# ZhengkunTian/OpenTransformer

Measured on AMD Instinct MI355X. Metric: utterances/sec (80-d fbank, ~1000 frames) train fwd+bwd, higher is better.
Workload: dtype fp16; 1 GPU; AISHELL-1 transformer_baseline.yaml (+input_size 80), 12 enc / 6 dec layers, B=32/GPU x 1000 frames x 80-d fbank, 15 decoder rows, V=4234, residual_dropout 0.1; step = fwd + bwd + grad all-reduce + clip/Adam/Noam; global_batch=32, frames=1000, parallelism=dp1, hipgraph=True

## Files before the change

### opentransformer_amd/csrc/common.h

```cpp
#pragma once
#include <hip/hip_runtime.h>
#include <stdint.h>

#include "../../include/otrans_hip.h"

#ifdef OTR_HALF_FP16
typedef _Float16 otr_hreal;
#define OTR_H16 OTR_F16
#else
typedef __bf16 otr_hreal;
#define OTR_H16 OTR_BF16
#endif
typedef __attribute__((ext_vector_type(8))) otr_hreal bf16x8;
typedef __attribute__((ext_vector_type(2))) otr_hreal bf16x2;
typedef __attribute__((ext_vector_type(4))) float f32x4;
typedef __attribute__((ext_vector_type(2))) float f32x2;
typedef uint16_t bf16_t;

void otr_set_error(const char* fmt, ...);
int32_t otr_check_launch(const char* what);
void otr_zero_f32(float* p, int64_t n, hipStream_t s);
#define OTR_REQUIRE(cond, ...)          \
  do {                                  \
    if (!(cond)) {                      \
      otr_set_error(__VA_ARGS__);       \
      return -1;                        \
    }                                   \
  } while (0)

extern int g_otr_force_tile;
extern int g_otr_force_ksplit;
extern int g_otr_conv2_wgrad256;
extern int g_otr_attn_enc96;
extern int g_otr_wgrad256;
extern int g_otr_wgrad256_grid;
extern int g_otr_conv2_dgrad_wide;
extern int g_otr_conv2_wide;
extern int g_otr_conv2_fwd_direct;
extern int g_otr_attn_enc;
extern int g_otr_attn_xmap;
extern int g_otr_attn_bwd_split;
extern int g_otr_beam_reg;
extern int g_otr_decode_attn64;
extern int g_otr_dec_group;
extern int g_otr_ffn_map;
extern int g_otr_ffn_coh_only;
extern int g_otr_spin_limit;
extern int32_t* g_otr_fault;
extern unsigned long long* g_otr_trace;

typedef uint32_t otr_u32x4 __attribute__((ext_vector_type(4)));
typedef uint32_t otr_u32x2 __attribute__((ext_vector_type(2)));
#define OTR_GLOBAL __attribute__((address_space(1)))
__device__ __forceinline__ uint4 ld_global_b128(const void* p) {
  otr_u32x4 v = *(const OTR_GLOBAL otr_u32x4*)(p);
  return make_uint4(v.x, v.y, v.z, v.w);
}
__device__ __forceinline__ uint2 ld_global_b64(const void* p) {
  otr_u32x2 v = *(const OTR_GLOBAL otr_u32x2*)(p);
  return make_uint2(v.x, v.y);
}
__device__ __forceinline__ void st_global_b128(void* p, uint4 v) {
  otr_u32x4 t = {v.x, v.y, v.z, v.w};
  *(OTR_GLOBAL otr_u32x4*)(p) = t;
}

__device__ __forceinline__ void st_global_b128_nt(void* p, uint4 v) {
  otr_u32x4 t = {v.x, v.y, v.z, v.w};
#if defined(OTR_ST_WT) && OTR_ST_WT
  asm volatile("global_store_dwordx4 %0, %1, off sc0 sc1 nt\n\ts_nop 1" ::"v"(p), "v"(t) : "memory");
#else
  __builtin_nontemporal_store(t, (OTR_GLOBAL otr_u32x4*)(p));
#endif
}

#ifdef OTR_HALF_FP16
__device__ __forceinline__ float bf2f(bf16_t v) { return (float)__builtin_bit_cast(_Float16, v); }
__device__ __forceinline__ float h2f_lo(uint32_t w) { return bf2f((bf16_t)(w & 0xffffu)); }
__device__ __forceinline__ float h2f_hi(uint32_t w) { return bf2f((bf16_t)(w >> 16)); }
#else
__device__ __forceinline__ float bf2f(bf16_t v) { return __uint_as_float(((uint32_t)v) << 16); }
__device__ __forceinline__ float h2f_lo(uint32_t w) { return __uint_as_float(w << 16); }
__device__ __forceinline__ float h2f_hi(uint32_t w) { return __uint_as_float(w & 0xffff0000u); }
#endif
__device__ __forceinline__ bf16_t f2bf(float f) {
  otr_hreal h = (otr_hreal)f;
  return __builtin_bit_cast(bf16_t, h);
}
__device__ __forceinline__ uint32_t pack2bf(float lo, float hi) {
  f32x2 v = {lo, hi};
  bf16x2 h = __builtin_convertvector(v, bf16x2);
  return __builtin_bit_cast(uint32_t, h);
}

__device__ __forceinline__ float h2f(bf16_t v) { return bf2f(v); }
__device__ __forceinline__ bf16_t f2h(float f) { return f2bf(f); }
__device__ __forceinline__ uint32_t pack2h(float lo, float hi) { return pack2bf(lo, hi); }

typedef __attribute__((ext_vector_type(16))) float f32x16;
__device__ __forceinline__ void mma32(f32x16& acc, const uint4& a, const uint4& b) {
#ifdef OTR_HALF_FP16
  acc = __builtin_amdgcn_mfma_f32_32x32x16_f16(__builtin_bit_cast(bf16x8, a), __builtin_bit_cast(bf16x8, b), acc, 0, 0, 0);
#else
  acc = __builtin_amdgcn_mfma_f32_32x32x16_bf16(__builtin_bit_cast(bf16x8, a), __builtin_bit_cast(bf16x8, b), acc, 0, 0, 0);
#endif
}

#ifdef OTR_HALF_FP16
#define OTR_MFMA32_OP "v_mfma_f32_32x32x16_f16"
#else
#define OTR_MFMA32_OP "v_mfma_f32_32x32x16_bf16"
#endif
__device__ __forceinline__ void mma32_agpr_b(f32x16& acc, const otr_u32x4& a, const otr_u32x4& b_acc) {
  asm volatile("s_nop 1\n\t" OTR_MFMA32_OP " %0, %1, %2, %0" : "+v"(acc) : "v"(a), "a"(b_acc));
}
__device__ __forceinline__ void mma32_agpr_a(f32x16& acc, const otr_u32x4& a_acc, const otr_u32x4& b) {
  asm volatile("s_nop 1\n\t" OTR_MFMA32_OP " %0, %1, %2, %0" : "+v"(acc) : "a"(a_acc), "v"(b));
}

typedef __attribute__((address_space(3))) unsigned char lds_byte;

template <bool NT = false> __device__ __forceinline__ void lds_dma(const void* src, uint32_t lds_dst) {
  uint32_t keep;
  if constexpr (NT)
    asm volatile("s_mov_b32 %0, m0\n\ts_mov_b32 m0, %2\n\ts_nop 0\n\tglobal_load_lds_dwordx4 %1, off nt\n\ts_mov_b32 m0, %0"
                 : "=&s"(keep) : "v"(src), "s"(lds_dst) : "memory");
  else
    asm volatile("s_mov_b32 %0, m0\n\ts_mov_b32 m0, %2\n\ts_nop 0\n\tglobal_load_lds_dwordx4 %1, off\n\ts_mov_b32 m0, %0"
                 : "=&s"(keep) : "v"(src), "s"(lds_dst) : "memory");
}
__device__ __forceinline__ void lds_dma_sbase(const void* uniform_src, uint32_t lane_off, uint32_t lds_dst) {
  uint32_t keep;
  asm volatile("s_mov_b32 %0, m0\n\ts_mov_b32 m0, %3\n\ts_nop 0\n\tglobal_load_lds_dwordx4 %1, %2\n\ts_mov_b32 m0, %0"
               : "=&s"(keep) : "v"(lane_off), "s"(uniform_src), "s"(lds_dst) : "memory");
}
template <int N> __device__ __forceinline__ void wait_vm() { asm volatile("s_waitcnt vmcnt(%0)" ::"n"(N) : "memory"); }
__device__ __forceinline__ void wait_lds() { asm volatile("s_waitcnt lgkmcnt(0)" ::: "memory"); }

constexpr int OTR_STAMP_BASE = 16384;
constexpr int OTR_KID_DECLAYER = 0, OTR_KID_ENCATTN = 6, OTR_KID_CONV2FWD = 9;
#define OTR_STAMP(TRACE, KID, UNIT, K, LIVE)                                                                    \
  do {                                                                                                          \
    if ((TRACE) && threadIdx.x == 0 && (LIVE))                                                                  \
      (TRACE)[OTR_STAMP_BASE + ((KID) * 256 + (UNIT)) * 16 + (K)] = __builtin_amdgcn_s_memtime();               \
  } while (0)

template <class T> struct ElemIO;
template <> struct ElemIO<float> {
  static __device__ __forceinline__ float ld(const float* p) { return *p; }
  static __device__ __forceinline__ void st(float* p, float v) { *p = v; }
};
template <> struct ElemIO<bf16_t> {
  static __device__ __forceinline__ float ld(const bf16_t* p) { return bf2f(*p); }
  static __device__ __forceinline__ void st(bf16_t* p, float v) { *p = f2bf(v); }
};

template <class CT> struct MMA;
template <> struct MMA<bf16_t> {
  static constexpr int CE = 8;
  static constexpr int KSTEP = 32;
  static constexpr int TPC = 2;
  static __device__ __forceinline__ void mma(f32x4& acc, const uint4& a, const uint4& b) {
#ifdef OTR_HALF_FP16
    acc = __builtin_amdgcn_mfma_f32_16x16x32_f16(__builtin_bit_cast(bf16x8, a), __builtin_bit_cast(bf16x8, b), acc, 0, 0, 0);
#else
    acc = __builtin_amdgcn_mfma_f32_16x16x32_bf16(__builtin_bit_cast(bf16x8, a), __builtin_bit_cast(bf16x8, b), acc, 0, 0, 0);
#endif
  }
  static __device__ __forceinline__ uint4 pack(const float* f) {
    uint4 r;
    r.x = pack2bf(f[0], f[1]);
    r.y = pack2bf(f[2], f[3]);
    r.z = pack2bf(f[4], f[5]);
    r.w = pack2bf(f[6], f[7]);
    return r;
  }
  static __device__ __forceinline__ uint4 from_tiles(const f32x4* t) {
    uint4 r;
    r.x = pack2bf(t[0][0], t[0][1]);
    r.y = pack2bf(t[0][2], t[0][3]);
    r.z = pack2bf(t[1][0], t[1][1]);
    r.w = pack2bf(t[1][2], t[1][3]);
    return r;
  }
};
template <> struct MMA<float> {
  static constexpr int CE = 4;
  static constexpr int KSTEP = 16;
  static constexpr int TPC = 1;
  static __device__ __forceinline__ void mma(f32x4& acc, const uint4& a, const uint4& b) {
    acc = __builtin_amdgcn_mfma_f32_16x16x4f32(__uint_as_float(a.x), __uint_as_float(b.x), acc, 0, 0, 0);
    acc = __builtin_amdgcn_mfma_f32_16x16x4f32(__uint_as_float(a.y), __uint_as_float(b.y), acc, 0, 0, 0);
    acc = __builtin_amdgcn_mfma_f32_16x16x4f32(__uint_as_float(a.z), __uint_as_float(b.z), acc, 0, 0, 0);
    acc = __builtin_amdgcn_mfma_f32_16x16x4f32(__uint_as_float(a.w), __uint_as_float(b.w), acc, 0, 0, 0);
  }
  static __device__ __forceinline__ uint4 pack(const float* f) {
    return make_uint4(__float_as_uint(f[0]), __float_as_uint(f[1]), __float_as_uint(f[2]), __float_as_uint(f[3]));
  }
  static __device__ __forceinline__ uint4 from_tiles(const f32x4* t) {
    return make_uint4(__float_as_uint(t[0][0]), __float_as_uint(t[0][1]), __float_as_uint(t[0][2]),
                      __float_as_uint(t[0][3]));
  }
};

template <class ST, int N>
__device__ __forceinline__ void load_row(const ST* p, int nvalid, bool vec, float* out) {
  if (vec && nvalid >= N) {
    if constexpr (sizeof(ST) == 4) {
#pragma unroll
      for (int i = 0; i < N; i += 4) {
        float4 v = *reinterpret_cast<const float4*>(p + i);
        out[i] = v.x; out[i + 1] = v.y; out[i + 2] = v.z; out[i + 3] = v.w;
      }
    } else {
      if constexpr (N == 8) {
        uint4 v = *reinterpret_cast<const uint4*>(p);
        out[0] = h2f_lo(v.x); out[1] = h2f_hi(v.x);
        out[2] = h2f_lo(v.y); out[3] = h2f_hi(v.y);
        out[4] = h2f_lo(v.z); out[5] = h2f_hi(v.z);
        out[6] = h2f_lo(v.w); out[7] = h2f_hi(v.w);
      } else {
        static_assert(N == 4, "bf16 rows are read 4 or 8 at a time");
        uint2 v = *reinterpret_cast<const uint2*>(p);
        out[0] = h2f_lo(v.x); out[1] = h2f_hi(v.x);
        out[2] = h2f_lo(v.y); out[3] = h2f_hi(v.y);
      }
    }
  } else {
#pragma unroll
    for (int i = 0; i < N; ++i) out[i] = (i < nvalid) ? ElemIO<ST>::ld(p + i) : 0.f;
  }
}

template <int NCH> __device__ __forceinline__ int swz(int row) {
  if constexpr (NCH == 4 || NCH == 12) return (0x78 >> (((row >> 2) & 3) * 2)) & 3;
  else if constexpr (NCH == 8) return (row >> 1) & 7;
  else if constexpr (NCH == 16) return row & 15;
  else return 0;
}

__device__ __forceinline__ float wave_sum(float v) {
#pragma unroll
  for (int o = 32; o > 0; o >>= 1) v += __shfl_xor(v, o);
  return v;
}
__device__ __forceinline__ float wave_max(float v) {
#pragma unroll
  for (int o = 32; o > 0; o >>= 1) v = fmaxf(v, __shfl_xor(v, o));
  return v;
}

__device__ __forceinline__ float pe_value(int t, int col, float neg_ln_over_d) {
  float div = expf((float)(col & ~1) * neg_ln_over_d);
  float ang = (float)t * div;
  return (col & 1) ? cosf(ang) : sinf(ang);
}

__device__ __forceinline__ uint32_t otr_rand32_sm64(uint64_t seed, uint64_t idx) {
  uint64_t z = seed + 0x9E3779B97F4A7C15ull * (idx + 1);
  z = (z ^ (z >> 30)) * 0xBF58476D1CE4E5B9ull;
  z = (z ^ (z >> 27)) * 0x94D049BB133111EBull;
  z = z ^ (z >> 31);
  return (uint32_t)(z >> 32);
}
__device__ __forceinline__ uint32_t otr_rand32(uint64_t seed, uint64_t idx) {
  const uint32_t s0 = (uint32_t)seed, s1 = (uint32_t)(seed >> 32);
  const uint32_t k0 = (s0 * 0x9E3779B1u) ^ s1;
  const uint32_t k1 = (s1 * 0x85EBCA77u) ^ (s0 >> 15) ^ 0xC2B2AE3Du;
  uint32_t x = (uint32_t)idx ^ k0;
  x += (uint32_t)(idx >> 32) * 0x27D4EB2Fu;
  x ^= x >> 16; x *= 0x7FEB352Du;
  x ^= x >> 15; x ^= k1; x *= 0x846CA68Bu;
  x ^= x >> 16;
  return x;
}

struct FastDiv {
  uint32_t d, magic, shift;
};
static inline FastDiv make_fastdiv(uint32_t d) {
  FastDiv f;
  f.d = d;
  if (d == 1) {
    f.magic = 0;
    f.shift = 0;
    return f;
  }
  uint32_t s = 0;
  while ((1u << s) < d) ++s;
  uint64_t m = ((1ull << (32 + s)) + d - 1) / d;
// ... 10 lines not shown
```

### opentransformer_amd/csrc/encattn.hip

```cpp
#include "tile32.h"

namespace {

constexpr int EA_T = 256;
constexpr int EA_TMAX = 512;
constexpr int EA_DK = 64;
constexpr int EA_HS = EA_DK * 2 + 16;
constexpr int EA_TS = EA_T * 2 + 8;
constexpr int EA_RM = EA_T * EA_HS;
constexpr int EA_TR = EA_DK * EA_TS;
constexpr float EA_LOG2E = 1.4426950408889634f;

struct EaArgs {
  unsigned long long* trace;
  const uint16_t *q, *k, *v, *o, *do_;
  uint16_t *dq, *dk, *dv;
  const uint8_t* key_mask;
  const float* lse;
  int B, H, T;
  int64_t q_bs, q_ts, k_bs, k_ts, v_bs, v_ts, o_bs, o_ts;
  float scale;
};


__device__ __forceinline__ uint4 ea_issue(const uint16_t* src, int64_t ts, int T, int tid, int c) {
  const int row = 64 * c + (tid >> 3);
  return ld_global_b128(src + (int64_t)min(row, T - 1) * ts + 8 * (tid & 7));
}
template <bool DOT>
__device__ __forceinline__ void ea_stage_rm(unsigned char* img, uint4 q, uint4 w, float* sdot, int T, int tid, int c) {
  const int row = 64 * c + (tid >> 3), ch = tid & 7;
  const uint32_t live = (uint32_t)0 - (uint32_t)(row < T);
  q.x &= live; q.y &= live; q.z &= live; q.w &= live;
  *reinterpret_cast<uint4*>(img + row * EA_HS + ch * 16) = q;
  if constexpr (DOT) {
    const uint32_t a[4] = {q.x, q.y, q.z, q.w}, b[4] = {w.x, w.y, w.z, w.w};
    float part = 0.f;
#pragma unroll
    for (int e = 0; e < 4; ++e) part += h2f_lo(a[e]) * h2f_lo(b[e]) + h2f_hi(a[e]) * h2f_hi(b[e]);
    part += __shfl_xor(part, 1);
    part += __shfl_xor(part, 2);
    part += __shfl_xor(part, 4);
    if (ch == 0) sdot[row] = part;
  }
}
__device__ __forceinline__ void ea_transpose(unsigned char* timg, const unsigned char* img, int c, int t, int e0, int ne) {
  const int rp = 32 * c + (t & 31), ch = (t >> 5) & 7;
  const uint4 a = *reinterpret_cast<const uint4*>(img + (2 * rp) * EA_HS + ch * 16);
  const uint4 b = *reinterpret_cast<const uint4*>(img + (2 * rp + 1) * EA_HS + ch * 16);
  const uint32_t aw[4] = {a.x, a.y, a.z, a.w}, bw[4] = {b.x, b.y, b.z, b.w};
#pragma unroll
  for (int e = 0; e < 4; ++e) {
    if (e < e0 || e >= e0 + ne) continue;
    *reinterpret_cast<uint32_t*>(timg + (8 * ch + 2 * e) * EA_TS + 4 * rp) = (aw[e] & 0xffffu) | (bw[e] << 16);
    *reinterpret_cast<uint32_t*>(timg + (8 * ch + 2 * e + 1) * EA_TS + 4 * rp) = (aw[e] >> 16) | (bw[e] & 0xffff0000u);
  }
}

__device__ __forceinline__ void ea_load_frags(uint4 (&f)[4], const uint16_t* src, int64_t ts, int row, int hi) {
#pragma unroll
  for (int ks = 0; ks < 4; ++ks) f[ks] = ld_global_b128(src + (int64_t)row * ts + 16 * ks + 8 * hi);
}

__device__ __forceinline__ void ea_put_rows(const f32x16 (&acc)[2], float scale, bool live, unsigned char* og, int lane) {
  const int m = lane & 31, hi = lane >> 5;
#pragma unroll
  for (int ct = 0; ct < 2; ++ct)
#pragma unroll
    for (int q = 0; q < 4; ++q) {
      uint2 v = make_uint2(pack2h(acc[ct][4 * q] * scale, acc[ct][4 * q + 1] * scale), pack2h(acc[ct][4 * q + 2] * scale, acc[ct][4 * q + 3] * scale));
      if (!live) v = make_uint2(0u, 0u);
      *reinterpret_cast<uint2*>(og + m * EA_HS + (32 * ct + 8 * q + 4 * hi) * 2) = v;
    }
}
__device__ __forceinline__ void ea_store_rows(const f32x16 (&acc)[2], float scale, bool live, unsigned char* og, uint16_t* dst, int64_t ts, int row0,
                                              int T, int lane) {
  ea_put_rows(acc, scale, live, og, lane);
  wait_lds();
#pragma unroll
  for (int q = 0; q < 4; ++q) {
    const int j = 8 * q + (lane >> 3), ch = lane & 7;
    if (row0 + j < T) st_global_b128(dst + (int64_t)(row0 + j) * ts + 8 * ch, *reinterpret_cast<const uint4*>(og + j * EA_HS + ch * 16));
  }
  wait_lds();
}

constexpr int EA_SMEM = 2 * EA_RM + 2 * EA_TR + 2 * EA_T * 4;

template <bool MULTI>
__global__ __launch_bounds__(512, 1) void encattn_bwd_kernel(EaArgs p) {
  __shared__ __attribute__((aligned(16))) unsigned char smem[EA_SMEM];
  const int tid = threadIdx.x, lane = tid & 63, m = lane & 31, hi = lane >> 5;
  const int wid = __builtin_amdgcn_readfirstlane(tid >> 6);
  const int xcd = (int)blockIdx.x & 7, kk = (int)blockIdx.x >> 3;
  const int T = p.T;
  const int nob = MULTI ? (T + EA_T - 1) / EA_T : 1;
  const int orient = kk & 1, ob = MULTI ? (kk >> 1) % nob : 0, g = (MULTI ? (kk >> 1) / nob : (kk >> 1)) * 8 + xcd;
  if (g >= p.H * p.B) return;
  const int h = g % p.H, b = g / p.H;
  const int o0 = ob * EA_T;
  const float sc2 = p.scale * EA_LOG2E;
  const uint16_t* Q = p.q + (int64_t)b * p.q_bs + h * EA_DK;
  const uint16_t* K = p.k + (int64_t)b * p.k_bs + h * EA_DK;
  const uint16_t* V = p.v + (int64_t)b * p.v_bs + h * EA_DK;
  const uint16_t* O = p.o + (int64_t)b * p.o_bs + h * EA_DK;
  const uint16_t* dO = p.do_ + (int64_t)b * p.o_bs + h * EA_DK;
  const float* lse = p.lse + ((int64_t)b * p.H + h) * T;
  const uint8_t* km = p.key_mask ? p.key_mask + (int64_t)b * T : nullptr;
  const int own = o0 + 32 * wid + m;
  const int ownc = min(own, T - 1);
  const bool wave_live = o0 + 32 * wid < T;
  OTR_STAMP(p.trace, OTR_KID_ENCATTN + orient, g, 0, g < 256);

  if (orient == 0) {
    unsigned char* krm = smem;
    unsigned char* vrm = smem + EA_RM;
    unsigned char* kt = smem + 2 * EA_RM;
    float* kbias = reinterpret_cast<float*>(smem + 2 * EA_RM + EA_TR);
    uint4 gk[4], gv[4], qf[4], dof[4], of[4];
    ea_load_frags(qf, Q, p.q_ts, ownc, hi);
    ea_load_frags(dof, dO, p.o_ts, ownc, hi);
    ea_load_frags(of, O, p.o_ts, ownc, hi);
    const float l0 = lse[ownc];
    uint8_t kmb = km ? km[min(tid, T - 1)] : (uint8_t)1;
#pragma unroll
    for (int c = 0; c < 4; ++c) {
      gk[c] = ea_issue(K, p.k_ts, T, tid, c);
      gv[c] = ea_issue(V, p.v_ts, T, tid, c);
    }
    __builtin_amdgcn_sched_barrier(0);
    OTR_STAMP(p.trace, OTR_KID_ENCATTN + orient, g, 1, g < 256);
    float del = 0.f;
#pragma unroll
    for (int ks = 0; ks < 4; ++ks) {
      const uint32_t a[4] = {dof[ks].x, dof[ks].y, dof[ks].z, dof[ks].w}, c[4] = {of[ks].x, of[ks].y, of[ks].z, of[ks].w};
#pragma unroll
      for (int e = 0; e < 4; ++e) del += h2f_lo(a[e]) * h2f_lo(c[e]) + h2f_hi(a[e]) * h2f_hi(c[e]);
    }
    del += __shfl_xor(del, 32);
    const float nl = (own < T && l0 != -__builtin_huge_valf()) ? -l0 * EA_LOG2E : -__builtin_huge_valf();
    f32x16 dq[2];
    tile_zero(dq[0]); tile_zero(dq[1]);
    auto tile = [&](int jt) {
      const unsigned char* kr = krm + jt * 32 * EA_HS;
      const unsigned char* vr = vrm + jt * 32 * EA_HS;
      f32x16 st, dp;
      tile_zero(st); tile_zero(dp);
#pragma unroll
      for (int ks = 0; ks < 4; ++ks) { mma32(st, frag_rm(kr, EA_HS, m, hi, ks), qf[ks]); mma32(dp, frag_rm(vr, EA_HS, m, hi, ks), dof[ks]); }
      float dsv[16];
#pragma unroll
      for (int q = 0; q < 4; ++q) {
        const float4 kb = *reinterpret_cast<const float4*>(kbias + jt * 32 + 8 * q + 4 * hi);
        const float kb4[4] = {kb.x, kb.y, kb.z, kb.w};
#pragma unroll
        for (int e = 0; e < 4; ++e) {
          const int r = 4 * q + e;
          const float pe = __builtin_amdgcn_exp2f(__builtin_fmaf(st[r], sc2, nl) + kb4[e]);
          dsv[r] = pe * (dp[r] - del);
        }
      }
#pragma unroll
      for (int k2 = 0; k2 < 2; ++k2) {
        const uint4 pb = frag_pack8(dsv + 8 * k2);
#pragma unroll
        for (int ct = 0; ct < 2; ++ct) mma32(dq[ct], frag_tr(kt, EA_TS, 32 * ct + m, jt * 32, hi, k2), pb);
      }
    };
    for (int s0 = 0; s0 < (MULTI ? T : 1); s0 += EA_T) {
      const int Ts = MULTI ? min(EA_T, T - s0) : T, nt = (Ts + 31) >> 5;
      if (MULTI && s0 > 0) {
        __syncthreads();
        kmb = km ? km[min(s0 + tid, T - 1)] : (uint8_t)1;
#pragma unroll
        for (int c = 0; c < 4; ++c) {
          gk[c] = ea_issue(K + (int64_t)s0 * p.k_ts, p.k_ts, Ts, tid, c);
          gv[c] = ea_issue(V + (int64_t)s0 * p.v_ts, p.v_ts, Ts, tid, c);
        }
      }
      if (tid < EA_T) kbias[tid] = (tid < Ts && kmb) ? 0.f : -__builtin_huge_valf();
#pragma unroll
      for (int c = 0; c < 4; ++c) {
        if (2 * c >= nt) break;
        ea_stage_rm<false>(krm, gk[c], gk[c], nullptr, Ts, tid, c);
        ea_stage_rm<false>(vrm, gv[c], gv[c], nullptr, Ts, tid, c);
        __syncthreads();
        ea_transpose(kt, krm, c, tid & 255, 2 * (tid >> 8), 2);
        __syncthreads();
        if (c == 0) OTR_STAMP(p.trace, OTR_KID_ENCATTN + orient, g, 2, g < 256);
        if (wave_live) {
          tile(2 * c);
          if (2 * c + 1 < nt) tile(2 * c + 1);
        }
      }
    }
    OTR_STAMP(p.trace, OTR_KID_ENCATTN + orient, g, 3, g < 256);
    __syncthreads();
    OTR_STAMP(p.trace, OTR_KID_ENCATTN + orient, g, 4, g < 256);
    if (wave_live) ea_store_rows(dq, p.scale, true, krm + 32 * wid * EA_HS, p.dq + (int64_t)b * p.q_bs + h * EA_DK, p.q_ts, o0 + 32 * wid, T, lane);
    OTR_STAMP(p.trace, OTR_KID_ENCATTN + orient, g, 5, g < 256);
  } else {
    unsigned char* qrm = smem;
    unsigned char* dorm = smem + EA_RM;
    unsigned char* qt = smem + 2 * EA_RM;
    unsigned char* dot = smem + 2 * EA_RM + EA_TR;
    float* nls = reinterpret_cast<float*>(smem + 2 * EA_RM + 2 * EA_TR);
    float* dels = nls + EA_T;
    uint4 gq[4], gdo[4], go[4], kf[4], vf[4];
    ea_load_frags(kf, K, p.k_ts, ownc, hi);
    ea_load_frags(vf, V, p.v_ts, ownc, hi);
    float l0 = lse[min(tid, T - 1)];
    const uint8_t kmb = km ? km[ownc] : (uint8_t)1;
#pragma unroll
    for (int c = 0; c < 4; ++c) {
      gq[c] = ea_issue(Q, p.q_ts, T, tid, c);
      gdo[c] = ea_issue(dO, p.o_ts, T, tid, c);
      go[c] = ea_issue(O, p.o_ts, T, tid, c);
    }
    __builtin_amdgcn_sched_barrier(0);
    OTR_STAMP(p.trace, OTR_KID_ENCATTN + orient, g, 1, g < 256);
    const bool keyok = own < T && kmb;
    f32x16 dk[2], dv[2];
    tile_zero(dk[0]); tile_zero(dk[1]); tile_zero(dv[0]); tile_zero(dv[1]);
    auto tile = [&](int it) {
      const unsigned char* qr = qrm + it * 32 * EA_HS;
      const unsigned char* dr = dorm + it * 32 * EA_HS;
      f32x16 st, dp;
      tile_zero(st); tile_zero(dp);
#pragma unroll
      for (int ks = 0; ks < 4; ++ks) { mma32(st, frag_rm(qr, EA_HS, m, hi, ks), kf[ks]); mma32(dp, frag_rm(dr, EA_HS, m, hi, ks), vf[ks]); }
      float pv[16], dsv[16];
#pragma unroll
      for (int q = 0; q < 4; ++q) {
        const float4 nl = *reinterpret_cast<const float4*>(nls + it * 32 + 8 * q + 4 * hi);
        const float4 de = *reinterpret_cast<const float4*>(dels + it * 32 + 8 * q + 4 * hi);
        const float nl4[4] = {nl.x, nl.y, nl.z, nl.w}, de4[4] = {de.x, de.y, de.z, de.w};
#pragma unroll
        for (int e = 0; e < 4; ++e) {
          const int r = 4 * q + e;
          pv[r] = __builtin_amdgcn_exp2f(__builtin_fmaf(st[r], sc2, nl4[e]));
          dsv[r] = pv[r] * (dp[r] - de4[e]);
        }
      }
#pragma unroll
      for (int k2 = 0; k2 < 2; ++k2) {
        const uint4 pb = frag_pack8(pv + 8 * k2), sb = frag_pack8(dsv + 8 * k2);
#pragma unroll
        for (int ct = 0; ct < 2; ++ct) {
          mma32(dv[ct], frag_tr(dot, EA_TS, 32 * ct + m, it * 32, hi, k2), pb);
          mma32(dk[ct], frag_tr(qt, EA_TS, 32 * ct + m, it * 32, hi, k2), sb);
        }
      }
    };
    for (int s0 = 0; s0 < (MULTI ? T : 1); s0 += EA_T) {
      const int Ts = MULTI ? min(EA_T, T - s0) : T, nt = (Ts + 31) >> 5;
      if (MULTI && s0 > 0) {
        __syncthreads();
        l0 = lse[min(s0 + tid, T - 1)];
#pragma unroll
        for (int c = 0; c < 4; ++c) {
          gq[c] = ea_issue(Q + (int64_t)s0 * p.q_ts, p.q_ts, Ts, tid, c);
          gdo[c] = ea_issue(dO + (int64_t)s0 * p.o_ts, p.o_ts, Ts, tid, c);
          go[c] = ea_issue(O + (int64_t)s0 * p.o_ts, p.o_ts, Ts, tid, c);
        }
      }
      if (tid < EA_T) nls[tid] = (tid < Ts && l0 != -__builtin_huge_valf()) ? -l0 * EA_LOG2E : -__builtin_huge_valf();
#pragma unroll
      for (int c = 0; c < 4; ++c) {
        if (2 * c >= nt) break;
        ea_stage_rm<false>(qrm, gq[c], gq[c], nullptr, Ts, tid, c);
        ea_stage_rm<true>(dorm, gdo[c], go[c], dels, Ts, tid, c);
        __syncthreads();
        if (tid < 256) ea_transpose(qt, qrm, c, tid, 0, 4);
        else ea_transpose(dot, dorm, c, tid - 256, 0, 4);
        __syncthreads();
        if (c == 0) OTR_STAMP(p.trace, OTR_KID_ENCATTN + orient, g, 2, g < 256);
        if (wave_live) {
          tile(2 * c);
          if (2 * c + 1 < nt) tile(2 * c + 1);
        }
      }
    }
    OTR_STAMP(p.trace, OTR_KID_ENCATTN + orient, g, 3, g < 256);
    __syncthreads();
    OTR_STAMP(p.trace, OTR_KID_ENCATTN + orient, g, 4, g < 256);
    if (wave_live) {
      ea_store_rows(dk, p.scale, keyok, qrm + 32 * wid * EA_HS, p.dk + (int64_t)b * p.k_bs + h * EA_DK, p.k_ts, o0 + 32 * wid, T, lane);
      ea_store_rows(dv, 1.f, keyok, dorm + 32 * wid * EA_HS, p.dv + (int64_t)b * p.v_bs + h * EA_DK, p.v_ts, o0 + 32 * wid, T, lane);
    }
    OTR_STAMP(p.trace, OTR_KID_ENCATTN + orient, g, 5, g < 256);
  }
}

}

bool encattn_bwd_takes(int dtype_is_h16, int dk, int Tq, int Tk, int causal, int has_bias, int vec) {
  return dtype_is_h16 && dk == EA_DK && Tq == Tk && Tq >= 1 && Tq <= EA_TMAX && !causal && !has_bias && vec;
}

int32_t encattn_bwd_launch(const void* q, const void* k, const void* v, const void* o, const void* do_, const float* lse, const uint8_t* key_mask,
                           void* dq, void* dk, void* dv, int B, int H, int T, int64_t q_bs, int64_t q_ts, int64_t k_bs, int64_t k_ts, int64_t v_bs,
                           int64_t v_ts, int64_t o_bs, int64_t o_ts, float scale, hipStream_t stream) {
  EaArgs p{};
  p.trace = g_otr_trace;
  p.q = (const uint16_t*)q; p.k = (const uint16_t*)k; p.v = (const uint16_t*)v; p.o = (const uint16_t*)o; p.do_ = (const uint16_t*)do_;
  p.dq = (uint16_t*)dq; p.dk = (uint16_t*)dk; p.dv = (uint16_t*)dv; p.key_mask = key_mask; p.lse = lse;
  p.B = B; p.H = H; p.T = T; p.q_bs = q_bs; p.q_ts = q_ts; p.k_bs = k_bs; p.k_ts = k_ts; p.v_bs = v_bs; p.v_ts = v_ts; p.o_bs = o_bs; p.o_ts = o_ts;
  p.scale = scale;
  if (T <= EA_T) {
    const unsigned grid = 8u * 2u * (unsigned)((H * B + 7) / 8);
    hipLaunchKernelGGL(encattn_bwd_kernel<false>, dim3(grid), dim3(512), 0, stream, p);
  } else {
    const unsigned nob = (unsigned)((T + EA_T - 1) / EA_T);
    const unsigned grid = 8u * 2u * nob * (unsigned)((H * B + 7) / 8);
    hipLaunchKernelGGL(encattn_bwd_kernel<true>, dim3(grid), dim3(512), 0, stream, p);
  }
  return otr_check_launch("encattn_bwd");
}
```

### opentransformer_amd/csrc/wgrad256.hip

```cpp
#include "common.h"
#include "wgrad256.h"

#include <algorithm>

namespace {

typedef short v4s __attribute__((ext_vector_type(4)));
typedef __attribute__((address_space(3))) v4s lds_v4s;

constexpr int SLAB_ROWS = 16;
constexpr int SLAB_BYTES = 16384;
constexpr int RING = 8, AHEAD = 6;
constexpr int LDS_BYTES = RING * SLAB_BYTES;

__device__ __forceinline__ uint2 tr_read(uint32_t lds_addr) {
  v4s r = __builtin_amdgcn_ds_read_tr16_b64_v4i16((lds_v4s*)(uintptr_t)lds_addr);
  return __builtin_bit_cast(uint2, r);
}

struct Frags {
  uint4 a[4], b[2];
};

__device__ __forceinline__ void read_frags_lo(Frags& f, uint32_t slab_addr, uint32_t a_off, uint32_t b_off) {
#pragma unroll
  for (int i = 0; i < 2; ++i) {
    const uint2 lo = tr_read(slab_addr + b_off + i * 512), hi = tr_read(slab_addr + b_off + 4096 + i * 512);
    f.b[i] = make_uint4(lo.x, lo.y, hi.x, hi.y);
  }
#pragma unroll
  for (int i = 0; i < 2; ++i) {
    const uint2 lo = tr_read(slab_addr + a_off + i * 512), hi = tr_read(slab_addr + a_off + 4096 + i * 512);
    f.a[i] = make_uint4(lo.x, lo.y, hi.x, hi.y);
  }
}
__device__ __forceinline__ void read_frags_hi(Frags& f, uint32_t slab_addr, uint32_t a_off, uint32_t b_off) {
#pragma unroll
  for (int i = 2; i < 4; ++i) {
    const uint2 lo = tr_read(slab_addr + a_off + i * 512), hi = tr_read(slab_addr + a_off + 4096 + i * 512);
    f.a[i] = make_uint4(lo.x, lo.y, hi.x, hi.y);
  }
}

__device__ __forceinline__ void frag_colsum(float (&cs)[4], const Frags& f) {
#ifdef OTR_HALF_FP16
  typedef _Float16 hv2 __attribute__((ext_vector_type(2)));
  const hv2 one = {(_Float16)1.f, (_Float16)1.f};
#define W256_DOT(w, c) __builtin_amdgcn_fdot2(__builtin_bit_cast(hv2, w), one, c, false)
#else
  typedef __bf16 hv2 __attribute__((ext_vector_type(2)));
  const hv2 one = {(__bf16)1.f, (__bf16)1.f};
#define W256_DOT(w, c) __builtin_amdgcn_fdot2_f32_bf16(__builtin_bit_cast(hv2, w), one, c, false)
#endif
#pragma unroll
  for (int a = 0; a < 4; ++a) {
    cs[a] = W256_DOT(f.a[a].x, cs[a]);
    cs[a] = W256_DOT(f.a[a].y, cs[a]);
    cs[a] = W256_DOT(f.a[a].z, cs[a]);
    cs[a] = W256_DOT(f.a[a].w, cs[a]);
  }
#undef W256_DOT
}

struct Stager {
  const unsigned char* base_a;
  const unsigned char* base_b;
  int64_t step_a, step_b;
  int row0, M;
  bool col_a, col_b;
  const unsigned char* zeros;
  uint32_t dst;
  int cT1, cF1, cT2, cF2, kh, kw;
  int64_t pix_bytes;
  FastDiv divF2, divT2;
  template <bool NTA, bool NTB, bool CONV = false> __device__ __forceinline__ void issue(int slab, int slot) {
    const bool ok = slab * SLAB_ROWS + row0 < M;
    const unsigned char* pa = ok && col_a ? base_a + slab * step_a : zeros;
    const unsigned char* pb;
    if constexpr (CONV) {
      const uint32_t m = (uint32_t)(slab * SLAB_ROWS + row0);
      const uint32_t t = fdiv(m, divF2), f2 = m - t * (uint32_t)cF2, b = fdiv(t, divT2), t2 = t - b * (uint32_t)cT2;
      const int fin = 2 * (int)f2 + kw - 1;
      const bool in = ok && col_b && fin >= 0 && fin < cF1;
      pb = in ? base_b + (((int64_t)b * cT1 + 2 * (int)t2 + kh) * cF1 + fin) * pix_bytes : zeros;
    } else {
      pb = ok && col_b ? base_b + slab * step_b : zeros;
    }
    lds_dma<NTA>(pa, (uint32_t)(slot * SLAB_BYTES) + dst);
    lds_dma<NTB>(pb, (uint32_t)(slot * SLAB_BYTES) + 8192u + dst);
  }
};

template <bool NTA, bool NTB, bool BIAS, bool CONV = false>
__device__ __forceinline__ void stream_piece(Stager& sg, f32x16 (&acc)[4][2], float (&cs)[4], int wc, int sb, int P, int rot,
                                             uint32_t a_off, uint32_t b_off) {
  int stage = rot;
  auto issue_next = [&](int slot) {
    sg.issue<NTA, NTB, CONV>(sb + stage, slot);
    stage = stage + 1 == P ? 0 : stage + 1;
  };
#pragma unroll
  for (int j = 0; j < AHEAD; ++j)
    if (j < P) issue_next(j);
  if (P >= AHEAD) wait_vm<2 * (AHEAD - 2)>(); else wait_vm<0>();
  __builtin_amdgcn_s_barrier();
  __builtin_amdgcn_sched_barrier(0);
  asm volatile("" ::: "memory");
  Frags f0, f1;
  read_frags_lo(f0, 0u, a_off, b_off);
  read_frags_hi(f0, 0u, a_off, b_off);
#define W256_MMA(A, CUR)                                                                                     \
  mma32(acc[A][0], CUR.a[A], CUR.b[0]);                                                                      \
  mma32(acc[A][1], CUR.a[A], CUR.b[1]);                                                                      \
  __builtin_amdgcn_sched_barrier(0);
#define W256_PHASE(Q, CUR, NXT, ST)                                                                          \
  {                                                                                                          \
    const int q_ = (Q);                                                                                      \
    const bool more_ = (ST) || q_ + AHEAD < P, next_ = (ST) || q_ + 1 < P;                      \
    const uint32_t nslab_ = (uint32_t)(((q_ + 1) & (RING - 1)) * SLAB_BYTES);                                \
    W256_MMA(0, CUR)                                                                                         \
    if (more_) issue_next((q_ + AHEAD) & (RING - 1));                                                        \
    __builtin_amdgcn_sched_barrier(0);                                                                       \
    W256_MMA(1, CUR)                                                                                         \
    if (next_) read_frags_lo(NXT, nslab_, a_off, b_off);                                                     \
    __builtin_amdgcn_sched_barrier(0);                                                                       \
    W256_MMA(2, CUR)                                                                                         \
    if (next_) read_frags_hi(NXT, nslab_, a_off, b_off);                                                     \
    __builtin_amdgcn_sched_barrier(0);                                                                       \
    W256_MMA(3, CUR)                                                                                         \
    if constexpr (BIAS) { if ((q_ & 3) == wc) frag_colsum(cs, CUR); }     \
    if (more_) wait_vm<2 * (AHEAD - 2)>(); else wait_vm<0>();                                                \
    __builtin_amdgcn_s_barrier();                                                                            \
    asm volatile("" ::: "memory");                                                                           \
    __builtin_amdgcn_sched_barrier(0);                                                                       \
  }
  int q = 0;
  for (; q + AHEAD + 1 < P; q += 2) {
    W256_PHASE(q, f0, f1, true)
    W256_PHASE(q + 1, f1, f0, true)
  }
  for (; q + 1 < P; q += 2) {
    W256_PHASE(q, f0, f1, false)
    W256_PHASE(q + 1, f1, f0, false)
  }
  if (q < P) W256_PHASE(q, f0, f1, false)
#undef W256_PHASE
#undef W256_MMA
}

template <bool COH, bool FIRST = false>
__device__ __forceinline__ void flush_tile(f32x16 (&acc)[4][2], float* dw, int ldw, int N, int K, int n_base, int k_base,
                                           unsigned char* scr, int lane) {
  constexpr int AUX = COH ? 17 : 0;
  const int rr = lane >> 3, cq = lane & 7;
  auto rs = __builtin_amdgcn_make_buffer_rsrc(dw, 0, ((N - 1) * ldw + K) * 4, 0x00020000);
#pragma unroll
  for (int h = 0; h < 2; ++h) {
    otr_u32x4 old[2][2][4];
    uint32_t off[2][2][4];
#pragma unroll
    for (int a2 = 0; a2 < 2; ++a2)
#pragma unroll
      for (int b = 0; b < 2; ++b)
#pragma unroll
        for (int j = 0; j < 4; ++j) {
          const int row = n_base + 32 * (2 * h + a2) + 8 * j + rr, col = k_base + 32 * b + 4 * cq;
          off[a2][b][j] = col < K ? (uint32_t)((row * ldw + col) * 4) : 0xfffffff0u;
          if constexpr (FIRST) old[a2][b][j] = otr_u32x4{0u, 0u, 0u, 0u};
          else old[a2][b][j] = __builtin_amdgcn_raw_buffer_load_b128(rs, off[a2][b][j], 0, AUX);
        }
#pragma unroll
// ... 359 lines not shown
```

Before: 7921 utterances/s.

## Use LDS transpose reads and software-pipeline staging in encoder attention backward

Removes the explicit LDS transpose images in the encoder attention backward kernel. Transposed operand fragments are now read directly from a new interleaved row-major LDS layout using ds_read_tr16, which frees LDS and drops one barrier plus the transpose pass per chunk. The tile loop is software-pipelined: the next tile's score MMA is issued inside the current step, and global loads for the next chunk are issued one chunk ahead with single-register prefetch, with sched_group_barrier pinning the interleave of MMA and VALU work. The risks are correctness of the new swizzled layout and added register pressure from the lookahead.

```diff
diff --git a/opentransformer_amd/csrc/common.h b/opentransformer_amd/csrc/common.h
--- a/opentransformer_amd/csrc/common.h
+++ b/opentransformer_amd/csrc/common.h
@@ -136,6 +136,13 @@
 }
 template <int N> __device__ __forceinline__ void wait_vm() { asm volatile("s_waitcnt vmcnt(%0)" ::"n"(N) : "memory"); }
 __device__ __forceinline__ void wait_lds() { asm volatile("s_waitcnt lgkmcnt(0)" ::: "memory"); }
+
+typedef short otr_v4s __attribute__((ext_vector_type(4)));
+typedef __attribute__((address_space(3))) otr_v4s otr_lds_v4s;
+__device__ __forceinline__ uint2 tr_read(uint32_t lds_addr) {
+  otr_v4s r = __builtin_amdgcn_ds_read_tr16_b64_v4i16((otr_lds_v4s*)(uintptr_t)lds_addr);
+  return __builtin_bit_cast(uint2, r);
+}
 
 constexpr int OTR_STAMP_BASE = 16384;
 constexpr int OTR_KID_DECLAYER = 0, OTR_KID_ENCATTN = 6, OTR_KID_CONV2FWD = 9;
diff --git a/opentransformer_amd/csrc/encattn.hip b/opentransformer_amd/csrc/encattn.hip
--- a/opentransformer_amd/csrc/encattn.hip
+++ b/opentransformer_amd/csrc/encattn.hip
@@ -6,10 +6,13 @@
 constexpr int EA_TMAX = 512;
 constexpr int EA_DK = 64;
 constexpr int EA_HS = EA_DK * 2 + 16;
-constexpr int EA_TS = EA_T * 2 + 8;
-constexpr int EA_RM = EA_T * EA_HS;
-constexpr int EA_TR = EA_DK * EA_TS;
+constexpr int EA_QS = 4 * EA_DK * 2 + 64 + 16;
+constexpr int EA_TILE = 8 * EA_QS;
+constexpr int EA_RM = (EA_T / 4) * EA_QS;
 constexpr float EA_LOG2E = 1.4426950408889634f;
+static_assert(EA_RM >= EA_T * EA_HS && EA_QS % 16 == 0, "the images double as output staging; rows stay 16-byte aligned");
+
+__device__ __forceinline__ int ea_row(int row) { return (row >> 2) * EA_QS + (row & 3) * (EA_DK * 2) + ((row >> 1) & 1) * 64; }
 
 struct EaArgs {
   unsigned long long* trace;
@@ -25,14 +28,15 @@
 
 __device__ __forceinline__ uint4 ea_issue(const uint16_t* src, int64_t ts, int T, int tid, int c) {
   const int row = 64 * c + (tid >> 3);
-  return ld_global_b128(src + (int64_t)min(row, T - 1) * ts + 8 * (tid & 7));
+  const uint32_t off = ((uint32_t)min(row, T - 1) * (uint32_t)ts + 8u * (uint32_t)(tid & 7)) * 2u;
+  return ld_global_b128(reinterpret_cast<const unsigned char*>(src) + off);
 }
 template <bool DOT>
 __device__ __forceinline__ void ea_stage_rm(unsigned char* img, uint4 q, uint4 w, float* sdot, int T, int tid, int c) {
   const int row = 64 * c + (tid >> 3), ch = tid & 7;
   const uint32_t live = (uint32_t)0 - (uint32_t)(row < T);
   q.x &= live; q.y &= live; q.z &= live; q.w &= live;
-  *reinterpret_cast<uint4*>(img + row * EA_HS + ch * 16) = q;
+  *reinterpret_cast<uint4*>(img + ea_row(row) + ch * 16) = q;
   if constexpr (DOT) {
     const uint32_t a[4] = {q.x, q.y, q.z, q.w}, b[4] = {w.x, w.y, w.z, w.w};
     float part = 0.f;
@@ -44,17 +48,16 @@
     if (ch == 0) sdot[row] = part;
   }
 }
-__device__ __forceinline__ void ea_transpose(unsigned char* timg, const unsigned char* img, int c, int t, int e0, int ne) {
-  const int rp = 32 * c + (t & 31), ch = (t >> 5) & 7;
-  const uint4 a = *reinterpret_cast<const uint4*>(img + (2 * rp) * EA_HS + ch * 16);
-  const uint4 b = *reinterpret_cast<const uint4*>(img + (2 * rp + 1) * EA_HS + ch * 16);
-  const uint32_t aw[4] = {a.x, a.y, a.z, a.w}, bw[4] = {b.x, b.y, b.z, b.w};
-#pragma unroll
-  for (int e = 0; e < 4; ++e) {
-    if (e < e0 || e >= e0 + ne) continue;
-    *reinterpret_cast<uint32_t*>(timg + (8 * ch + 2 * e) * EA_TS + 4 * rp) = (aw[e] & 0xffffu) | (bw[e] << 16);
-    *reinterpret_cast<uint32_t*>(timg + (8 * ch + 2 * e + 1) * EA_TS + 4 * rp) = (aw[e] >> 16) | (bw[e] & 0xffff0000u);
-  }
+
+__device__ __forceinline__ uint4 ea_frag_rm(const unsigned char* tile, int rm, int ks) {
+  return *reinterpret_cast<const uint4*>(tile + rm + 32 * ks);
+}
+__device__ __forceinline__ int ea_tr_lane(int lane) {
+  return (lane >> 5) * EA_QS + ea_row((lane & 15) >> 2) + 32 * ((lane >> 4) & 1) + 8 * (lane & 3);
+}
+__device__ __forceinline__ uint4 ea_frag_tr(uint32_t tile_tr, int k2, int ct) {
+  const uint2 lo = tr_read(tile_tr + 4 * k2 * EA_QS + 64 * ct), up = tr_read(tile_tr + (4 * k2 + 2) * EA_QS + 64 * ct);
+  return make_uint4(lo.x, lo.y, up.x, up.y);
 }
 
 __device__ __forceinline__ void ea_load_frags(uint4 (&f)[4], const uint16_t* src, int64_t ts, int row, int hi) {
@@ -85,7 +88,22 @@
   wait_lds();
 }
 
-constexpr int EA_SMEM = 2 * EA_RM + 2 * EA_TR + 2 * EA_T * 4;
+__device__ __forceinline__ int ea_lane() { return (int)__builtin_amdgcn_mbcnt_hi(~0u, __builtin_amdgcn_mbcnt_lo(~0u, 0u)); }
+
+constexpr int EA_SMEM = 2 * EA_RM + 2 * EA_T * 4;
+
+template <int NC> __device__ __forceinline__ void ea_pin_step() {
+#pragma unroll
+  for (int i = 0; i < 8; ++i) {
+    __builtin_amdgcn_sched_group_barrier(0x008, 1, 0);
+    __builtin_amdgcn_sched_group_barrier(0x002, 5, 0);
+  }
+#pragma unroll
+  for (int i = 0; i < NC; ++i) {
+    __builtin_amdgcn_sched_group_barrier(0x008, 1, 0);
+    __builtin_amdgcn_sched_group_barrier(0x002, 40 / NC, 0);
+  }
+}
 
 template <bool MULTI>
 __global__ __launch_bounds__(512, 1) void encattn_bwd_kernel(EaArgs p) {
@@ -110,24 +128,21 @@
   const int own = o0 + 32 * wid + m;
   const int ownc = min(own, T - 1);
   const bool wave_live = o0 + 32 * wid < T;
+  const int rm = ea_row(m) + 16 * hi;
+  const uint32_t tr = (uint32_t)(uintptr_t)(lds_byte*)smem + (uint32_t)ea_tr_lane(lane);
   OTR_STAMP(p.trace, OTR_KID_ENCATTN + orient, g, 0, g < 256);
 
   if (orient == 0) {
     unsigned char* krm = smem;
     unsigned char* vrm = smem + EA_RM;
-    unsigned char* kt = smem + 2 * EA_RM;
-    float* kbias = reinterpret_cast<float*>(smem + 2 * EA_RM + EA_TR);
-    uint4 gk[4], gv[4], qf[4], dof[4], of[4];
+    float* kbias = reinterpret_cast<float*>(smem + 2 * EA_RM);
+    uint4 gk, gv, qf[4], dof[4], of[4];
     ea_load_frags(qf, Q, p.q_ts, ownc, hi);
     ea_load_frags(dof, dO, p.o_ts, ownc, hi);
     ea_load_frags(of, O, p.o_ts, ownc, hi);
     const float l0 = lse[ownc];
     uint8_t kmb = km ? km[min(tid, T - 1)] : (uint8_t)1;
-#pragma unroll
-    for (int c = 0; c < 4; ++c) {
-      gk[c] = ea_issue(K, p.k_ts, T, tid, c);
-      gv[c] = ea_issue(V, p.v_ts, T, tid, c);
-    }
+    gk = ea_issue(K, p.k_ts, T, tid, 0); gv = ea_issue(V, p.v_ts, T, tid, 0);
     __builtin_amdgcn_sched_barrier(0);
     OTR_STAMP(p.trace, OTR_KID_ENCATTN + orient, g, 1, g < 256);
     float del = 0.f;
@@ -141,152 +156,174 @@
     const float nl = (own < T && l0 != -__builtin_huge_valf()) ? -l0 * EA_LOG2E : -__builtin_huge_valf();
     f32x16 dq[2];
     tile_zero(dq[0]); tile_zero(dq[1]);
-    auto tile = [&](int jt) {
-      const unsigned char* kr = krm + jt * 32 * EA_HS;
-      const unsigned char* vr = vrm + jt * 32 * EA_HS;
-      f32x16 st, dp;
-      tile_zero(st); tile_zero(dp);
-#pragma unroll
-      for (int ks = 0; ks < 4; ++ks) { mma32(st, frag_rm(kr, EA_HS, m, hi, ks), qf[ks]); mma32(dp, frag_rm(vr, EA_HS, m, hi, ks), dof[ks]); }
-      float dsv[16];
-#pragma unroll
-      for (int q = 0; q < 4; ++q) {
-        const float4 kb = *reinterpret_cast<const float4*>(kbias + jt * 32 + 8 * q + 4 * hi);
-        const float kb4[4] = {kb.x, kb.y, kb.z, kb.w};
-#pragma unroll
-        for (int e = 0; e < 4; ++e) {
-          const int r = 4 * q + e;
-          const float pe = __builtin_amdgcn_exp2f(__builtin_fmaf(st[r], sc2, nl) + kb4[e]);
-          dsv[r] = pe * (dp[r] - del);
-        }
-      }
+    auto front = [&](int jt, f32x16& st) {
+      const unsigned char* kr = krm + jt * EA_TILE;
+      tile_zero(st);
+#pragma unroll
+      for (int ks = 0; ks < 4; ++ks) mma32(st, ea_frag_rm(kr, rm, ks), qf[ks]);
+    };
+    auto step = [&](int jt, int jn, const f32x16& st, f32x16& stn) {
+      __builtin_amdgcn_sched_barrier(0);
+      const unsigned char* vr = vrm + jt * EA_TILE;
+      f32x16 dp;
+      tile_zero(dp);
+#pragma unroll
+      for (int ks = 0; ks < 4; ++ks) mma32(dp, ea_frag_rm(vr, rm, ks), dof[ks]);
+      front(jn, stn);
+      const uint32_t kt = tr + jt * EA_TILE;
 #pragma unroll
       for (int k2 = 0; k2 < 2; ++k2) {
-        const uint4 pb = frag_pack8(dsv + 8 * k2);
-#pragma unroll
-        for (int ct = 0; ct < 2; ++ct) mma32(dq[ct], frag_tr(kt, EA_TS, 32 * ct + m, jt * 32, hi, k2), pb);
-      }
+        float dsv[8], kb[8];
+#pragma unroll
+        for (int q = 0; q < 2; ++q) {
+          const float4 k4 = *reinterpret_cast<const float4*>(kbias + jt * 32 + 16 * k2 + 8 * q + 4 * hi);
+          kb[4 * q] = k4.x; kb[4 * q + 1] = k4.y; kb[4 * q + 2] = k4.z; kb[4 * q + 3] = k4.w;
+        }
+#pragma unroll
+        for (int e = 0; e < 8; ++e) {
+          const int r = 8 * k2 + e;
+          const float pe = __builtin_amdgcn_exp2f(__builtin_fmaf(st[r], sc2, nl) + kb[e]);
+          dsv[e] = pe * (dp[r] - del);
+        }
+        const uint4 pb = frag_pack8(dsv);
+#pragma unroll
+        for (int ct = 0; ct < 2; ++ct) mma32(dq[ct], ea_frag_tr(kt, k2, ct), pb);
+      }
+      ea_pin_step<2>();
+      __builtin_amdgcn_sched_barrier(0);
     };
     for (int s0 = 0; s0 < (MULTI ? T : 1); s0 += EA_T) {
       const int Ts = MULTI ? min(EA_T, T - s0) : T, nt = (Ts + 31) >> 5;
+      const uint16_t* Ks = K + (int64_t)s0 * p.k_ts;
+      const uint16_t* Vs = V + (int64_t)s0 * p.v_ts;
       if (MULTI && s0 > 0) {
         __syncthreads();
         kmb = km ? km[min(s0 + tid, T - 1)] : (uint8_t)1;
-#pragma unroll
-        for (int c = 0; c < 4; ++c) {
-          gk[c] = ea_issue(K + (int64_t)s0 * p.k_ts, p.k_ts, Ts, tid, c);
-          gv[c] = ea_issue(V + (int64_t)s0 * p.v_ts, p.v_ts, Ts, tid, c);
-        }
+        gk = ea_issue(Ks, p.k_ts, Ts, tid, 0); gv = ea_issue(Vs, p.v_ts, Ts, tid, 0);
       }
       if (tid < EA_T) kbias[tid] = (tid < Ts && kmb) ? 0.f : -__builtin_huge_valf();
-#pragma unroll
-      for (int c = 0; c < 4; ++c) {
-        if (2 * c >= nt) break;
-        ea_stage_rm<false>(krm, gk[c], gk[c], nullptr, Ts, tid, c);
-        ea_stage_rm<false>(vrm, gv[c], gv[c], nullptr, Ts, tid, c);
-        __syncthreads();
-        ea_transpose(kt, krm, c, tid & 255, 2 * (tid >> 8), 2);
-        __syncthreads();
-        if (c == 0) OTR_STAMP(p.trace, OTR_KID_ENCATTN + orient, g, 2, g < 256);
-        if (wave_live) {
-          tile(2 * c);
-          if (2 * c + 1 < nt) tile(2 * c + 1);
-        }
+      ea_stage_rm<false>(krm, gk, gk, nullptr, Ts, tid, 0);
+      ea_stage_rm<false>(vrm, gv, gv, nullptr, Ts, tid, 0);
+      gk = ea_issue(Ks, p.k_ts, Ts, tid, 1); gv = ea_issue(Vs, p.v_ts, Ts, tid, 1);
+      __syncthreads();
+      if (s0 == 0) OTR_STAMP(p.trace, OTR_KID_ENCATTN + orient, g, 2, g < 256);
+      f32x16 sa, sb;
+      if (wave_live) front(0, sa);
+      for (int c = 0; 2 * c < nt; ++c) {
+        const bool has1 = 2 * c + 1 < nt, next = 2 * c + 2 < nt;
+        if (wave_live) step(2 * c, has1 ? 2 * c + 1 : 2 * c, sa, sb);
+        if (!has1) break;
+        if (next) {
+          ea_stage_rm<false>(krm, gk, gk, nullptr, Ts, tid, c + 1);
+          ea_stage_rm<false>(vrm, gv, gv, nullptr, Ts, tid, c + 1);
+          if (2 * c + 4 < nt) { gk = ea_issue(Ks, p.k_ts, Ts, tid, c + 2); gv = ea_issue(Vs, p.v_ts, Ts, tid, c + 2); }
+          __syncthreads();
+        }
+        if (wave_live) step(2 * c + 1, next ? 2 * c + 2 : 2 * c + 1, sb, sa);
       }
     }
     OTR_STAMP(p.trace, OTR_KID_ENCATTN + orient, g, 3, g < 256);
     __syncthreads();
     OTR_STAMP(p.trace, OTR_KID_ENCATTN + orient, g, 4, g < 256);
-    if (wave_live) ea_store_rows(dq, p.scale, true, krm + 32 * wid * EA_HS, p.dq + (int64_t)b * p.q_bs + h * EA_DK, p.q_ts, o0 + 32 * wid, T, lane);
+    if (wave_live) ea_store_rows(dq, p.scale, true, krm + 32 * wid * EA_HS, p.dq + (int64_t)b * p.q_bs + h * EA_DK, p.q_ts, o0 + 32 * wid, T, ea_lane());
     OTR_STAMP(p.trace, OTR_KID_ENCATTN + orient, g, 5, g < 256);
   } else {
     unsigned char* qrm = smem;
     unsigned char* dorm = smem + EA_RM;
-    unsigned char* qt = smem + 2 * EA_RM;
-    unsigned char* dot = smem + 2 * EA_RM + EA_TR;
-    float* nls = reinterpret_cast<float*>(smem + 2 * EA_RM + 2 * EA_TR);
+    float* nls = reinterpret_cast<float*>(smem + 2 * EA_RM);
     float* dels = nls + EA_T;
-    uint4 gq[4], gdo[4], go[4], kf[4], vf[4];
+    uint4 gq, gdo, go, kf[4], vf[4];
     ea_load_frags(kf, K, p.k_ts, ownc, hi);
     ea_load_frags(vf, V, p.v_ts, ownc, hi);
     float l0 = lse[min(tid, T - 1)];
     const uint8_t kmb = km ? km[ownc] : (uint8_t)1;
-#pragma unroll
-    for (int c = 0; c < 4; ++c) {
-      gq[c] = ea_issue(Q, p.q_ts, T, tid, c);
-      gdo[c] = ea_issue(dO, p.o_ts, T, tid, c);
-      go[c] = ea_issue(O, p.o_ts, T, tid, c);
-    }
+    gq = ea_issue(Q, p.q_ts, T, tid, 0); gdo = ea_issue(dO, p.o_ts, T, tid, 0); go = ea_issue(O, p.o_ts, T, tid, 0);
     __builtin_amdgcn_sched_barrier(0);
     OTR_STAMP(p.trace, OTR_KID_ENCATTN + orient, g, 1, g < 256);
     const bool keyok = own < T && kmb;
     f32x16 dk[2], dv[2];
     tile_zero(dk[0]); tile_zero(dk[1]); tile_zero(dv[0]); tile_zero(dv[1]);
-    auto tile = [&](int it) {
-      const unsigned char* qr = qrm + it * 32 * EA_HS;
-      const unsigned char* dr = dorm + it * 32 * EA_HS;
-      f32x16 st, dp;
-      tile_zero(st); tile_zero(dp);
-#pragma unroll
-      for (int ks = 0; ks < 4; ++ks) { mma32(st, frag_rm(qr, EA_HS, m, hi, ks), kf[ks]); mma32(dp, frag_rm(dr, EA_HS, m, hi, ks), vf[ks]); }
-      float pv[16], dsv[16];
-#pragma unroll
-      for (int q = 0; q < 4; ++q) {
-        const float4 nl = *reinterpret_cast<const float4*>(nls + it * 32 + 8 * q + 4 * hi);
-        const float4 de = *reinterpret_cast<const float4*>(dels + it * 32 + 8 * q + 4 * hi);
-        const float nl4[4] = {nl.x, nl.y, nl.z, nl.w}, de4[4] = {de.x, de.y, de.z, de.w};
-#pragma unroll
-        for (int e = 0; e < 4; ++e) {
-          const int r = 4 * q + e;
-          pv[r] = __builtin_amdgcn_exp2f(__builtin_fmaf(st[r], sc2, nl4[e]));
-          dsv[r] = pv[r] * (dp[r] - de4[e]);
-        }
-      }
+    auto front = [&](int it, f32x16& st) {
+      const unsigned char* qr = qrm + it * EA_TILE;
+      tile_zero(st);
+#pragma unroll
+      for (int ks = 0; ks < 4; ++ks) mma32(st, ea_frag_rm(qr, rm, ks), kf[ks]);
+    };
+    auto step = [&](int it, int in, const f32x16& st, f32x16& stn) {
+      __builtin_amdgcn_sched_barrier(0);
+      const unsigned char* dr = dorm + it * EA_TILE;
+      f32x16 dp;
+      tile_zero(dp);
+#pragma unroll
+      for (int ks = 0; ks < 4; ++ks) mma32(dp, ea_frag_rm(dr, rm, ks), vf[ks]);
+      front(in, stn);
+      const uint32_t qt = tr + it * EA_TILE, dot = qt + EA_RM;
 #pragma unroll
       for (int k2 = 0; k2 < 2; ++k2) {
-        const uint4 pb = frag_pack8(pv + 8 * k2), sb = frag_pack8(dsv + 8 * k2);
+        float pv[8], dsv[8], nlv[8], dev[8];
+#pragma unroll
+        for (int q = 0; q < 2; ++q) {
+          const float4 nl = *reinterpret_cast<const float4*>(nls + it * 32 + 16 * k2 + 8 * q + 4 * hi);
+          const float4 de = *reinterpret_cast<const float4*>(dels + it * 32 + 16 * k2 + 8 * q + 4 * hi);
+          nlv[4 * q] = nl.x; nlv[4 * q + 1] = nl.y; nlv[4 * q + 2] = nl.z; nlv[4 * q + 3] = nl.w;
+          dev[4 * q] = de.x; dev[4 * q + 1] = de.y; dev[4 * q + 2] = de.z; dev[4 * q + 3] = de.w;
+        }
+#pragma unroll
+        for (int e = 0; e < 8; ++e) {
+          const int r = 8 * k2 + e;
+          pv[e] = __builtin_amdgcn_exp2f(__builtin_fmaf(st[r], sc2, nlv[e]));
+          dsv[e] = pv[e] * (dp[r] - dev[e]);
+        }
+        const uint4 pb = frag_pack8(pv), sb = frag_pack8(dsv);
 #pragma unroll
         for (int ct = 0; ct < 2; ++ct) {
-          mma32(dv[ct], frag_tr(dot, EA_TS, 32 * ct + m, it * 32, hi, k2), pb);
-          mma32(dk[ct], frag_tr(qt, EA_TS, 32 * ct + m, it * 32, hi, k2), sb);
-        }
-      }
+          mma32(dv[ct], ea_frag_tr(dot, k2, ct), pb);
+          mma32(dk[ct], ea_frag_tr(qt, k2, ct), sb);
+        }
+      }
+      ea_pin_step<4>();
+      __builtin_amdgcn_sched_barrier(0);
     };
     for (int s0 = 0; s0 < (MULTI ? T : 1); s0 += EA_T) {
       const int Ts = MULTI ? min(EA_T, T - s0) : T, nt = (Ts + 31) >> 5;
+      const uint16_t* Qs = Q + (int64_t)s0 * p.q_ts;
+      const uint16_t* dOs = dO + (int64_t)s0 * p.o_ts;
+      const uint16_t* Os = O + (int64_t)s0 * p.o_ts;
       if (MULTI && s0 > 0) {
         __syncthreads();
         l0 = lse[min(s0 + tid, T - 1)];
-#pragma unroll
-        for (int c = 0; c < 4; ++c) {
-          gq[c] = ea_issue(Q + (int64_t)s0 * p.q_ts, p.q_ts, Ts, tid, c);
-          gdo[c] = ea_issue(dO + (int64_t)s0 * p.o_ts, p.o_ts, Ts, tid, c);
-          go[c] = ea_issue(O + (int64_t)s0 * p.o_ts, p.o_ts, Ts, tid, c);
-        }
+        gq = ea_issue(Qs, p.q_ts, Ts, tid, 0); gdo = ea_issue(dOs, p.o_ts, Ts, tid, 0); go = ea_issue(Os, p.o_ts, Ts, tid, 0);
       }
       if (tid < EA_T) nls[tid] = (tid < Ts && l0 != -__builtin_huge_valf()) ? -l0 * EA_LOG2E : -__builtin_huge_valf();
-#pragma unroll
-      for (int c = 0; c < 4; ++c) {
-        if (2 * c >= nt) break;
-        ea_stage_rm<false>(qrm, gq[c], gq[c], nullptr, Ts, tid, c);
-        ea_stage_rm<true>(dorm, gdo[c], go[c], dels, Ts, tid, c);
-        __syncthreads();
-        if (tid < 256) ea_transpose(qt, qrm, c, tid, 0, 4);
-        else ea_transpose(dot, dorm, c, tid - 256, 0, 4);
-        __syncthreads();
-        if (c == 0) OTR_STAMP(p.trace, OTR_KID_ENCATTN + orient, g, 2, g < 256);
-        if (wave_live) {
-          tile(2 * c);
-          if (2 * c + 1 < nt) tile(2 * c + 1);
-        }
+      ea_stage_rm<false>(qrm, gq, gq, nullptr, Ts, tid, 0);
+      ea_stage_rm<true>(dorm, gdo, go, dels, Ts, tid, 0);
+      gq = ea_issue(Qs, p.q_ts, Ts, tid, 1); gdo = ea_issue(dOs, p.o_ts, Ts, tid, 1); go = ea_issue(Os, p.o_ts, Ts, tid, 1);
+      __syncthreads();
+      if (s0 == 0) OTR_STAMP(p.trace, OTR_KID_ENCATTN + orient, g, 2, g < 256);
+      f32x16 sa, sb;
+      if (wave_live) front(0, sa);
+      for (int c = 0; 2 * c < nt; ++c) {
+        const bool has1 = 2 * c + 1 < nt, next = 2 * c + 2 < nt;
+        if (wave_live) step(2 * c, has1 ? 2 * c + 1 : 2 * c, sa, sb);
+        if (!has1) break;
+        if (next) {
+          ea_stage_rm<false>(qrm, gq, gq, nullptr, Ts, tid, c + 1);
+          ea_stage_rm<true>(dorm, gdo, go, dels, Ts, tid, c + 1);
+          if (2 * c + 4 < nt) {
+            gq = ea_issue(Qs, p.q_ts, Ts, tid, c + 2); gdo = ea_issue(dOs, p.o_ts, Ts, tid, c + 2); go = ea_issue(Os, p.o_ts, Ts, tid, c + 2);
+          }
+          __syncthreads();
+        }
+        if (wave_live) step(2 * c + 1, next ? 2 * c + 2 : 2 * c + 1, sb, sa);
       }
     }
     OTR_STAMP(p.trace, OTR_KID_ENCATTN + orient, g, 3, g < 256);
     __syncthreads();
     OTR_STAMP(p.trace, OTR_KID_ENCATTN + orient, g, 4, g < 256);
     if (wave_live) {
-      ea_store_rows(dk, p.scale, keyok, qrm + 32 * wid * EA_HS, p.dk + (int64_t)b * p.k_bs + h * EA_DK, p.k_ts, o0 + 32 * wid, T, lane);
-      ea_store_rows(dv, 1.f, keyok, dorm + 32 * wid * EA_HS, p.dv + (int64_t)b * p.v_bs + h * EA_DK, p.v_ts, o0 + 32 * wid, T, lane);
+      const int le = ea_lane();
+      ea_store_rows(dk, p.scale, keyok, qrm + 32 * wid * EA_HS, p.dk + (int64_t)b * p.k_bs + h * EA_DK, p.k_ts, o0 + 32 * wid, T, le);
+      ea_store_rows(dv, 1.f, keyok, dorm + 32 * wid * EA_HS, p.dv + (int64_t)b * p.v_bs + h * EA_DK, p.v_ts, o0 + 32 * wid, T, le);
     }
     OTR_STAMP(p.trace, OTR_KID_ENCATTN + orient, g, 5, g < 256);
   }
diff --git a/opentransformer_amd/csrc/wgrad256.hip b/opentransformer_amd/csrc/wgrad256.hip
--- a/opentransformer_amd/csrc/wgrad256.hip
+++ b/opentransformer_amd/csrc/wgrad256.hip
@@ -4,19 +4,11 @@
 #include <algorithm>
 
 namespace {
-
-typedef short v4s __attribute__((ext_vector_type(4)));
-typedef __attribute__((address_space(3))) v4s lds_v4s;
 
 constexpr int SLAB_ROWS = 16;
 constexpr int SLAB_BYTES = 16384;
 constexpr int RING = 8, AHEAD = 6;
 constexpr int LDS_BYTES = RING * SLAB_BYTES;
-
-__device__ __forceinline__ uint2 tr_read(uint32_t lds_addr) {
-  v4s r = __builtin_amdgcn_ds_read_tr16_b64_v4i16((lds_v4s*)(uintptr_t)lds_addr);
-  return __builtin_bit_cast(uint2, r);
-}
 
 struct Frags {
   uint4 a[4], b[2];
```

After: 7951 utterances/s, median of 6. Within noise of the previous version (+0.4%).
